# kieranrcampbell/clonealign

Measured on AMD Instinct MI355X. Metric: ELBO iterations/sec, higher is better.
Workload: dtype f32 variables (contraction: float64 series over gene bins; count-matrix products: int8 MFMA, exact); 1 GPU; synthetic 100000 cells x 5000 genes x 8 clones, K=1, S=1, cell-sharded over 1 GPU(s) (BASELINE.json configs[2]); cells=100000, genes=5000, clones=8, K=1, mc_samples=1, y_storage=u8, y_bytes_per_elem=1, fused_sweep=True, fwd_mfma=True, series_form=True, y_mfma=True, parallelism=single, collective=none, allreduce_doubles_per_train_pass=20764, build_id=88308988739b5500

## Files before the change

clonealign_amd/csrc/ca_eng_loop.inc:

```
int wait_y(ca_engine* h, bool all) {
  if (all) {
    if (h->y_pending) HIPCK(h, hipStreamWaitEvent(h->stream, h->ev_ydone, 0));
    h->y_pending = false; h->yw_pending = false;
  } else if (h->yw_pending) {
    HIPCK(h, hipStreamWaitEvent(h->stream, h->ev_ywdone, 0));
    h->yw_pending = false;
  }
  return CA_OK;
}

int make_etamax(ca_engine* h) {
  if (h->D > 0) {
    LAUNCH(h, CA_KERNEL_OTHER, hipLaunchKernelGGL(k_vmm_final, dim3(1), dim3(64), 0, h->stream, h->vmm_part, h->vmm, h->ngblk, h->D));
    LAUNCH(h, CA_KERNEL_OTHER, hipLaunchKernelGGL(k_etamax, dim3(cdiv(h->N, CA_TB)), dim3(CA_TB), 0, h->stream, h->F, h->vmm, h->etamax2, h->N, h->D));
  }
  h->em_stale = false;
  return CA_OK;
}
int ensure_etamax(ca_engine* h) {
  if (!h->em_stale) return CA_OK;
  return make_etamax(h);
}

int refresh_derived(ca_engine* h) {
// ... 69 lines not shown
                                                  h->V, h->D, (int64_t)h->G, h->F, h->D, h->N, 1, h->ys_amax));
  }
  LAUNCH(h, CA_KERNEL_OTHER, hipLaunchKernelGGL(k_ys_quant, dim3(a.nblk), dim3(CA_YM_TB), 0, h->stream, a));
  return CA_OK;
}
ca_ys_io ys_io(ca_engine* h) {
  ca_ys_io io;
  io.Wr = h->Wr; io.Pr = h->Pr; io.Wsum = h->Wsum; io.Psum = h->Psum; io.exps = h->ys_exps + 2 * h->ys_slot;
  io.YWpart = h->YWpart; io.YTpart = h->YTpart;
  io.esc_off = h->ys4 ? h->esc_off : nullptr; io.esc = h->ys4 ? h->esc : nullptr;
  io.perm = nullptr;
  return io;
}
ca_ovf_args ys_ovf(ca_engine* h) { return ovf_args(h, h->YWpart + (int64_t)h->ys_nseg * h->N); }
int yfin_flush(ca_engine* h) {
  if (!h->yfin_pending) return CA_OK;
  h->yfin_pending = false;
  return launch_yfinish(h, h->ys_nrg, h->ys_nseg);
}
int ys_finish(ca_engine* h, bool defer = false) {
  h->yfin_pending = true;
  if (!defer) CACK(yfin_flush(h));
  h->ys_slot = (h->ys_slot + 1) % 3;
  h->ys_steps = 0;
  h->ys_quant_ready = false;
  h->ycache_valid = true;
  return CA_OK;
}
template <bool Y4, int N2 = 0>
void launch_ys(ca_engine* h) {
  constexpr int lds = Y4 ? CA_YS4_LDS_BYTES : CA_YS_LDS_BYTES;
  ca_ys_io yio = ys_io(h);
  const uint8_t* Yimg = h->Ys;
  if (N2 > 0) { Yimg = h->Ys2; yio.esc_off = h->esc2_off; yio.esc = h->esc2; yio.perm = h->y2_perm; }
  const int nb_main = h->ys_nrg * h->ys_nseg;
  const ca_pm_args* pm = h->mom_args;
  h->mom_args = nullptr;
  const int nmom = pm ? pm->nmb + pm->nred : 0;
  if (h->n_ovf > 0) {
    const ca_ovf_args ovf = ys_ovf(h);
    const dim3 grid(nmom + nb_main + ovf.nb_rows + ovf.nb_chunks);
    if (pm) {
      ca_pm_args pmo = *pm;
      if (h->mom_last && h->mom_ovf_first) pmo.blk0 += ovf.nb_rows + ovf.nb_chunks;
      hipLaunchKernelGGL((k_ys_mfma_ovf_mom<Y4, N2>), grid, dim3(CA_YM_TB), lds, h->stream, Yimg, yio, h->N, h->Gp, h->ys_RS, nb_main, ovf, h->F, h->V, h->D, pmo);
    }
// ... 847 lines not shown
```

clonealign_amd/csrc/ca_eng_state.inc:

```
namespace {

thread_local std::string g_last_error;

typedef struct { char internal[128]; } ca_nccl_uid;
typedef void* ca_nccl_comm;
struct RcclApi {
  void* lib = nullptr;
  int (*GetUniqueId)(ca_nccl_uid*) = nullptr;
  int (*CommInitRank)(ca_nccl_comm*, int, ca_nccl_uid, int) = nullptr;
  int (*CommDestroy)(ca_nccl_comm) = nullptr;
  int (*AllReduce)(const void*, void*, size_t, int, int, ca_nccl_comm, hipStream_t) = nullptr;
  const char* (*GetErrorString)(int) = nullptr;
  std::string err;
  bool load() {
    if (lib) return true;
    const char* cands[] = {getenv("CLONEALIGN_RCCL_LIB"), "librccl.so.1", "librccl.so", "/opt/rocm/lib/librccl.so.1",
                           "/opt/rocm/lib/librccl.so"};
    for (const char* c : cands) {
      if (!c || !*c) continue;
      lib = dlopen(c, RTLD_NOW | RTLD_LOCAL);
      if (lib) break;
    }
    if (!lib) { err = std::string("cannot dlopen librccl: ") + dlerror(); return false; }
    GetUniqueId = (decltype(GetUniqueId))dlsym(lib, "ncclGetUniqueId");
// ... 130 lines not shown
  bool tail_fuse = true;
  double* host_dev = nullptr;
  unsigned long long host_seq = 0, host_seq_next = 0;
  float* eps_stage = nullptr; size_t eps_stage_bytes = 0;
  hipEvent_t ev_stage = nullptr;
  bool fwd_cell = false; int ncblk_f = 0, fc_tl = 4;
  int fc_nbig = 0;
  bool fwd_mfma = false; int fsplit = 1, fkchunk = 1, nk32 = 1; unsigned short* Mq = nullptr;
  bool fwd_bal = false; int bal_q = 0, bal_r = 0, bal_nchunk = 0; unsigned long long* bal_xw = nullptr; unsigned bal_tag = 0;
  bool pfwd = false; int pf_npair = 0, pf_fsplit = 1, pf_kchunk = 1; unsigned short* pf_Mq = nullptr; float* pf_Z = nullptr;
  int bwd_pairs = 0;
  bool bwd_mfma = false, bwd_frac = false, c16 = false, s2 = false, s2f = false;
  unsigned short* coefq = nullptr; int64_t N16 = 0, cchunk_m = 0; int csplit_m = 1, nwt = 0;
  int bwd_tl = CA_BWD_TL;
  uint64_t draw = 0;
  hipEvent_t ev_ywdone = nullptr; bool yw_pending = false, on_side = false;
  bool y_ys = false, ys4 = false; int* esc_off = nullptr; unsigned* esc = nullptr; int64_t n_esc = 0;
  int ys_n2 = 0; uint8_t* Ys2 = nullptr; unsigned short *y2_perm = nullptr, *y2_pos = nullptr; int* esc2_off = nullptr; unsigned* esc2 = nullptr; int64_t n_esc2 = 0;
  uint8_t* Ys = nullptr; uint4 *Wr = nullptr, *Pr = nullptr; int *Wsum = nullptr, *Psum = nullptr;
  int* ys_exps = nullptr;
  unsigned* ys_amax = nullptr;
  float* ys_amaxp = nullptr; int ys_nq = 0;
  int ys_ncap = 0, ys_namax[3] = {0, 0, 0};
  bool ys_quant_ready = false;
  int ys_slot = 0, ys_steps = -1, ys_RS = 256, ys_nrg = 0, ys_nseg = 0; int64_t ys_N64 = 0; float ys_step_bound = -1.f;
  double adam_bound = -1.0;
  ca_p2p* p2p = nullptr;
  ca_nccl_comm comm = nullptr;
  ca_host_allreduce_fn host_ar = nullptr; void* host_ar_user = nullptr; double* host_ar_buf = nullptr; int64_t host_ar_cap = 0;
  std::vector<EvPair> ev_pool; size_t ev_used = 0; bool prof_open = false;
  unsigned prof_seen[CA_KERNEL_COUNT] = {0, 0, 0, 0, 0};
  double k_ms[CA_KERNEL_COUNT] = {0}; int64_t k_n[CA_KERNEL_COUNT] = {0};
  int n_cu = 256;
};

namespace {

#define HIPCK(h, call)                                                                       \
  do {                                                                                       \
    hipError_t e_ = (call);                                                                  \
    if (e_ != hipSuccess) {                                                                  \
      (h)->err = std::string(#call) + ": " + hipGetErrorString(e_);                          \
      return CA_ERR_HIP;                                                                     \
    }                                                                                        \
  } while (0)

// ... 321 lines not shown
```

clonealign_amd/csrc/ca_ymfma.hip.h:

```cpp
#pragma once
#include <hip/hip_runtime.h>
#include <stdint.h>

typedef int ca_i32x4 __attribute__((ext_vector_type(4)));

#define CA_YM_TB 256

__device__ __forceinline__ int ca_fix_exp(float amax) { return amax > 0.f ? 29 - ilogbf(amax) : 0; }

__global__ void __launch_bounds__(CA_YM_TB) k_ym_absmax(const float* __restrict__ V, int Dv, int64_t G, const float* __restrict__ F, int Df,
                                                        int64_t N, int K, unsigned* __restrict__ amax) {
  const int64_t i = (int64_t)blockIdx.x * CA_YM_TB + threadIdx.x;
  float mw = 0.f, mp = 0.f;
  if (i < G) for (int k = 0; k < K; ++k) mw = fmaxf(mw, fabsf(V[i * Dv + k]));
  if (i < N) for (int k = 0; k < K; ++k) mp = fmaxf(mp, fabsf(F[i * Df + k]));
#pragma unroll
  for (int o = 32; o > 0; o >>= 1) { mw = fmaxf(mw, __shfl_xor(mw, o, 64)); mp = fmaxf(mp, __shfl_xor(mp, o, 64)); }
  if ((threadIdx.x & 63) == 0) {
    if (i < G + 64) atomicMax(amax, __float_as_uint(mw));
    if (i < N + 64) atomicMax(amax + 1, __float_as_uint(mp));
  }
}
__device__ __forceinline__ int ca_digit(int x, int p) {
  int d = 0;
// ... 162 lines not shown
        const unsigned y = n < N ? col[n * (int64_t)Gp] : 0u;
        x |= (y < 3u ? y : 3u) << (2 * t);
      }
    } else {
#pragma unroll
      for (int t = 0; t < 2; ++t) {
        const int64_t n = cs * 64 + 32 * ld + 16 * t + j;
        const unsigned y = n < N ? col[n * (int64_t)Gp] : 0u;
        x |= (y < 15u ? y : 15u) << (4 * t);
      }
    }
    w[gb >> 2] |= x << (8 * (gb & 3));
  }
  Y2[i] = (uint4){w[0], w[1], w[2], w[3]};
}

__device__ __forceinline__ ca_i32x4 ca_mfma_i8(uint4 a, uint4 b, ca_i32x4 c) {
  return __builtin_amdgcn_mfma_i32_16x16x64_i8(__builtin_bit_cast(ca_i32x4, a), __builtin_bit_cast(ca_i32x4, b), c, 0, 0, 0);
}

constexpr int CA_YS_GW = 512;
static_assert(CA_YS_GW == 512, "k_ys_mfma's accumulator switch has eight cases");
constexpr int CA_YS_PITCH = 80;

__device__ __forceinline__ void ca_ds_read_tr_b8_x8(unsigned addr, uint2 (&lo)[4], uint2 (&hi)[4]) {
  asm volatile(
      "ds_read_b64_tr_b8 %0, %8\n\tds_read_b64_tr_b8 %4, %8 offset:640\n\t"
      "ds_read_b64_tr_b8 %1, %8 offset:16\n\tds_read_b64_tr_b8 %5, %8 offset:656\n\t"
      "ds_read_b64_tr_b8 %2, %8 offset:32\n\tds_read_b64_tr_b8 %6, %8 offset:672\n\t"
      "ds_read_b64_tr_b8 %3, %8 offset:48\n\tds_read_b64_tr_b8 %7, %8 offset:688\n\t"
      "s_waitcnt lgkmcnt(0)"
      : "=&v"(lo[0]), "=&v"(lo[1]), "=&v"(lo[2]), "=&v"(lo[3]), "=&v"(hi[0]), "=&v"(hi[1]), "=&v"(hi[2]), "=&v"(hi[3])
      : "v"(addr)
      : "memory");
}
__device__ __forceinline__ void ca_ds_read_tr_b8_x4(unsigned addr, uint2 (&lo)[2], uint2 (&hi)[2]) {
  asm volatile(
      "ds_read_b64_tr_b8 %0, %4\n\tds_read_b64_tr_b8 %2, %4 offset:640\n\t"
      "ds_read_b64_tr_b8 %1, %4 offset:16\n\tds_read_b64_tr_b8 %3, %4 offset:656\n\t"
      "s_waitcnt lgkmcnt(0)"
      : "=&v"(lo[0]), "=&v"(lo[1]), "=&v"(hi[0]), "=&v"(hi[1])
      : "v"(addr)
      : "memory");
}
static_assert(8 * CA_YS_PITCH == 640, "offsets in ca_ds_read_tr_b8_x8 / _x4 assume the 80-byte pitch");
__device__ __forceinline__ uint4 ca_and4(uint4 a, unsigned m) { return (uint4){a.x & m, a.y & m, a.z & m, a.w & m}; }

#ifndef CA_YS_DEPTH
#define CA_YS_DEPTH 2
#endif
#ifndef CA_YS_WAVES
#define CA_YS_WAVES 3
#endif
struct ca_ys_io {
  const uint4* Wr; const uint4* Pr; const int* Wsum; const int* Psum; const int* exps;
  float* YWpart; float* YTpart;
  const int* esc_off; const unsigned* esc;
  const unsigned short* perm;
};
#ifndef CA_YS4_DEPTH
#define CA_YS4_DEPTH 4
#endif
#ifndef CA_YS4_WAVES
#define CA_YS4_WAVES 4
#endif
constexpr int CA_YS4_OFF_W = 4 * 64 * CA_YS_PITCH;
constexpr int CA_YS4_OFF_ROW = CA_YS4_OFF_W + (CA_YS_GW / 64) * 1024;
constexpr int CA_YS4_OFF_PSI = CA_YS4_OFF_ROW + 4 * 64 * 8;
constexpr int CA_YS4_OFF_COL = 4 * (CA_YS_GW / 64) * 64 * 4 * 4;
constexpr int CA_YS4_LDS_BYTES = CA_YS4_OFF_COL + CA_YS_GW * 8;
static_assert(CA_YS4_OFF_PSI + 4 * 256 <= CA_YS4_OFF_COL, "the 4-bit launch's tables fit below its column-escape sums");
static_assert(4 * CA_YS4_LDS_BYTES <= 160 * 1024, "four blocks of the 4-bit launch per CU");
template <int DEPTH = CA_YS_DEPTH, bool Y4 = false, bool OWN = false, int N2 = 0>
__device__ __forceinline__ void ca_ys_mfma_body(int blk, const uint8_t* __restrict__ Ys, const ca_ys_io& io, int64_t N, int Gp,
                                                int RS ,
                                                unsigned char* ca_ys_lds ) {
  const uint4* __restrict__ Wr = io.Wr;
  const uint4* __restrict__ Pr = io.Pr;
  constexpr bool Y4L = Y4 && OWN;
  constexpr int NP = CA_YS_GW / 64;
  static_assert(NP % DEPTH == 0, "pieces per cell step must be a multiple of the pipeline depth");
  static_assert(N2 == 0 || (Y4 && OWN && N2 < NP), "the 2-bit blocks belong to the 4-bit image's own launch");
  constexpr int SB2 = N2 * 1024 + (NP - N2) * 2048;
  const int lane = threadIdx.x & 63, j = lane & 15, q = lane >> 4;
  const int wv = __builtin_amdgcn_readfirstlane((int)(threadIdx.x >> 6) & 3);
  const int nseg = Gp / CA_YS_GW;
  const int rg = blk / nseg, seg = blk - rg * nseg;
  unsigned char* my = ca_ys_lds + (size_t)wv * 64 * CA_YS_PITCH;
  const int64_t c0 = ((int64_t)rg * 4 + wv) * RS;
  const int64_t c1 = (c0 + RS < N) ? c0 + RS : N;
  const int g0 = seg * CA_YS_GW;
  const unsigned grp = (unsigned)(j >> 2);
  unsigned msk[4];
#pragma unroll
  for (int t = 0; t < 4; ++t) msk[t] = grp == (unsigned)t ? 0xFFFFFFFFu : 0u;
  ca_i32x4 acc_yt[NP];
#pragma unroll
  for (int a = 0; a < NP; ++a) acc_yt[a] = (ca_i32x4){0, 0, 0, 0};
  const int lrow = lane >> 2, lch = lane & 3;
  unsigned char* wr_dst = my + lrow * CA_YS_PITCH + 16 * lch;
  const unsigned char* rd_row = my + j * CA_YS_PITCH + 16 * q;
  const unsigned rd_tr = (unsigned)(size_t)my + (unsigned)((16 * q + (j >> 1)) * CA_YS_PITCH + 8 * (j & 1));
  constexpr int PB = Y4 ? 2048 : 4096, NL = PB / 1024;
  const uint8_t* src = N2 > 0 ? Ys + ((c0 >> 6) * (int64_t)nseg + seg) * SB2
                              : Ys + ((c0 >> 6) * (int64_t)(Gp / 64) + (g0 >> 6)) * PB;
  const uint4* wsrc = Wr + (int64_t)(g0 >> 6) * 64;
  const unsigned voff = 16u * (unsigned)lane;
  uint4 R[DEPTH][NL], W[DEPTH];
  const int nsteps = c0 < c1 ? (int)((c1 - c0 + 63) / 64) : 0;
  typedef unsigned ca_v4u __attribute__((ext_vector_type(4)));
  const __amdgpu_buffer_rsrc_t ry = __builtin_amdgcn_make_buffer_rsrc(const_cast<uint8_t*>(src), 0, 0x7FFFFFFF, 0x00020000);
  const __amdgpu_buffer_rsrc_t rw = __builtin_amdgcn_make_buffer_rsrc(const_cast<uint4*>(wsrc), 0, NP * 1024, 0x00020000);
  const __amdgpu_buffer_rsrc_t rp = __builtin_amdgcn_make_buffer_rsrc(const_cast<uint4*>(Pr + (c0 >> 6) * 64), 0, 0x7FFFFFFF, 0x00020000);
  auto issue = [&](int slot, int st, int a, unsigned vo) {
    const int so = N2 > 0 ? st * nseg * SB2 + (a < N2 ? a * 1024 : N2 * 1024 + (a - N2) * 2048) : (st * (Gp / 64) + a) * PB;
#pragma unroll
    for (int i = 0; i < NL; ++i) {
      if (N2 > 0 && i > 0 && a < N2) continue;
      const ca_v4u v = __builtin_amdgcn_raw_buffer_load_b128(ry, (int)(vo + 1024u * (unsigned)i), so, 2 );
      R[slot][i] = (uint4){v.x, v.y, v.z, v.w};
    }
    if (!Y4L) {
      const ca_v4u w = __builtin_amdgcn_raw_buffer_load_b128(rw, (int)voff, a * 1024, 0);
      W[slot] = (uint4){w.x, w.y, w.z, w.w};
    }
  };
  uint4* wl = reinterpret_cast<uint4*>(ca_ys_lds + CA_YS4_OFF_W);
  unsigned long long* colesc = reinterpret_cast<unsigned long long*>(ca_ys_lds + CA_YS4_OFF_COL);
  uint4 wimg[2], pidx[2][2];
  int eoff = 0;
  if (Y4L) {
    wimg[0] = wsrc[threadIdx.x];
    wimg[1] = wsrc[threadIdx.x + CA_YM_TB];
    if (N2 > 0) {
#pragma unroll
      for (int h2 = 0; h2 < 2; ++h2) {
        const uint4* pq = reinterpret_cast<const uint4*>(io.perm + g0 + 16 * (((int)threadIdx.x + h2 * CA_YM_TB) >> 4));
        pidx[h2][0] = pq[0]; pidx[h2][1] = pq[1];
      }
    }
    if (lane <= nsteps) eoff = io.esc_off[((int64_t)blk * 4 + wv) * RS + (64 * lane < RS ? 64 * lane : RS)];
  }
// ... 25 lines not shown
          w4[b >> 2] |= (unsigned)tb[((gi >> 6) * 64 + 16 * ((gi >> 4) & 3)) * 16 + (gi & 15)] << (8 * (b & 3));
        }
        wimg[h2] = (uint4){w4[0], w4[1], w4[2], w4[3]};
      }
    }
    wl[threadIdx.x] = wimg[0];
    wl[threadIdx.x + CA_YM_TB] = wimg[1];
    colesc[threadIdx.x] = 0ull;
    colesc[threadIdx.x + CA_YM_TB] = 0ull;
    __syncthreads();
  }
  ca_i32x4 acc_yw[4];
  uint4 prm[4];
  int wtot[4] = {0, 0, 0, 0};
  if (!Y4) {
    const int* ws = io.Wsum + (g0 >> 6) * 4;
#pragma unroll
    for (int a = 0; a < NP; ++a)
#pragma unroll
      for (int p_ = 0; p_ < 4; ++p_) wtot[p_] += ws[a * 4 + p_];
  }
  const int e_w = io.exps[0];
  const int64_t kb = ((int64_t)blk * 4 + wv) * RS;
  unsigned long long* rowesc = reinterpret_cast<unsigned long long*>(ca_ys_lds + (Y4L ? CA_YS4_OFF_ROW : 4 * 64 * CA_YS_PITCH)) + wv * 64;
  unsigned char* psl = ca_ys_lds + CA_YS4_OFF_PSI + wv * 256;
  if (Y4) rowesc[lane] = 0ull;
  for (int st = 0; st < nsteps; ++st) {
    const int64_t cs = c0 + (int64_t)st * 64;
    const bool more = st + 1 < nsteps;
    uint4 pr;
    if (Y4L) {
      pr = pr_nx;
#pragma unroll
      for (int t = 0; t < 4; ++t) acc_yw[t] = (ca_i32x4){0, 0, 0, 0};
    } else {
      const ca_v4u pv = __builtin_amdgcn_raw_buffer_load_b128(rp, (int)voff, st * 1024, 0);
      pr = (uint4){pv.x, pv.y, pv.z, pv.w};
#pragma unroll
      for (int t = 0; t < 4; ++t) { acc_yw[t] = (ca_i32x4){0, 0, 0, 0}; if (!Y4L) prm[t] = ca_and4(pr, msk[t]); }
    }
    int e_lo = 0, e_hi = 0;
    unsigned en0 = 0u, en1 = 0u;
    if (Y4L) {
      e_lo = __builtin_amdgcn_readlane(eoff, st);
      e_hi = __builtin_amdgcn_readlane(eoff, st + 1);
      if (e_hi > e_lo) {
        en0 = io.esc[e_lo + lane < e_hi ? e_lo + lane : e_hi - 1];
        en1 = io.esc[e_lo + 64 + lane < e_hi ? e_lo + 64 + lane : e_hi - 1];
      }
    }
#pragma unroll
    for (int a = 0; a < NP; ++a) {
      const int slot = a % DEPTH;
      __builtin_amdgcn_sched_barrier(0);
      const uint4 wr = Y4L ? wl[a * 64 + lane] : W[slot];
      if (Y4) {
#pragma unroll
        for (int t = 0; t < 4; ++t) {
          const bool nar = N2 > 0 && a < N2;
          const uint4 v = R[slot][nar ? 0 : t >> 1];
          const int sh = nar ? 2 * t : 4 * (t & 1);
          const uint4 av = ca_and4((uint4){v.x >> sh, v.y >> sh, v.z >> sh, v.w >> sh}, nar ? 0x03030303u : 0x0F0F0F0Fu);
          *reinterpret_cast<uint4*>(const_cast<unsigned char*>(rd_row) + 16 * t * CA_YS_PITCH) = av;
          acc_yw[t] = ca_mfma_i8(av, wr, acc_yw[t]);
        }
        if (a + DEPTH < NP) issue(slot, st, a + DEPTH, voff);
        else if (Y4L) {
          const unsigned vo = more ? voff : 0x80000000u + voff;
          if (a + DEPTH == NP) {
            const ca_v4u pv = __builtin_amdgcn_raw_buffer_load_b128(rp, (int)vo, (st + 1) * 1024, 0);
            pr_nx = (uint4){pv.x, pv.y, pv.z, pv.w};
          }
          issue(slot, st + 1, a + DEPTH - NP, vo);
        } else if (more) issue(slot, st + 1, a + DEPTH - NP, voff);
      } else {
#pragma unroll
        for (int i = 0; i < 4; ++i) *reinterpret_cast<uint4*>(wr_dst + 16 * i * CA_YS_PITCH) = R[slot][i];
        if (a + DEPTH < NP) issue(slot, st, a + DEPTH, voff);
        else if (more) issue(slot, st + 1, a + DEPTH - NP, voff);
#pragma unroll
        for (int t = 0; t < 4; ++t) {
          const uint4 av = *reinterpret_cast<const uint4*>(rd_row + 16 * t * CA_YS_PITCH);
          acc_yw[t] = ca_mfma_i8(av, wr, acc_yw[t]);
        }
      }
#pragma unroll
      for (int h2 = 0; h2 < 2; ++h2) {
        uint2 lo[2], hi[2];
        ca_ds_read_tr_b8_x4(rd_tr + 32u * (unsigned)h2, lo, hi);
#pragma unroll
        for (int t = 0; t < 2; ++t) {
          uint4 pa;
          if (Y4L) {
            unsigned g_ = grp;
            asm volatile("" : "+v"(g_));
            pa = ca_and4(pr, g_ == (unsigned)(2 * h2 + t) ? 0xFFFFFFFFu : 0u);
          } else {
            pa = prm[2 * h2 + t];
          }
          acc_yt[a] = ca_mfma_i8(pa, (uint4){lo[t].x, lo[t].y, hi[t].x, hi[t].y}, acc_yt[a]);
        }
      }
    }
    if (Y4L) {
      if (j < 4) *reinterpret_cast<uint4*>(psl + (4 * q + j) * 16) = pr;
      const unsigned char* wlb = reinterpret_cast<const unsigned char*>(wl);
      auto esc1 = [&](unsigned en) {
        const int c = (int)(en & 63u), gi = (int)((en >> 9) & 511u);
        const unsigned char* dw = wlb + ((gi >> 6) * 64 + 16 * ((gi >> 4) & 3)) * 16 + (gi & 15);
        const unsigned char* dp = psl + 64 * (c >> 4) + (c & 15);
        unsigned fw = 0u, fp = 0u;
#pragma unroll
        for (int p_ = 0; p_ < 4; ++p_) {
          fw += (unsigned)(int)(signed char)dw[16 * p_] << (8 * p_);
          fp += (unsigned)(int)(signed char)dp[16 * p_] << (8 * p_);
        }
        const long long x = (long long)(en >> 18);
        atomicAdd(rowesc + c, (unsigned long long)(x * (long long)(int)fw));
        atomicAdd(colesc + gi, (unsigned long long)(x * (long long)(int)fp));
// ... 60 lines not shown
    }
  }
  const double inv_p = ldexp(1.0, -io.exps[1]);
  for (int i = (int)threadIdx.x & (CA_YM_TB - 1); i < NP * 64; i += CA_YM_TB) {
    const int l = i & 63, a = i >> 6;
    double v = 0.0;
#pragma unroll
    for (int r = 3; r >= 0; --r) {
      const int o = i * 4 + r;
      const int sr = (comb[o] + comb[o + NP * 256]) + (comb[o + 2 * NP * 256] + comb[o + 3 * NP * 256]);
      v = v * 256.0 + (double)((long long)sr + 128 * pb[r]);
    }
    const int gl = 16 * (4 * a + (l >> 4)) + (l & 15), gene = g0 + (N2 > 0 ? (int)io.perm[g0 + gl] : gl);
    if (Y4L) v += (double)(long long)colesc[gl];
    io.YTpart[(int64_t)rg * Gp + gene] = (float)(v * inv_p);
  }
}
template <bool Y4, int N2 = 0>
__global__ void __launch_bounds__(CA_YM_TB, Y4 ? CA_YS4_WAVES : CA_YS_WAVES) k_ys_mfma(const uint8_t* __restrict__ Ys, ca_ys_io io, int64_t N, int Gp, int RS) {
  extern __shared__ __attribute__((aligned(16))) unsigned char ca_ys_dyn[];
  ca_ys_mfma_body<Y4 ? CA_YS4_DEPTH : CA_YS_DEPTH, Y4, true, N2>((int)blockIdx.x, Ys, io, N, Gp, RS, ca_ys_dyn);
}
constexpr int CA_YS_LDS_BYTES = 4 * (CA_YS_GW / 64) * 64 * 4 * 4;
static_assert(4 * 64 * CA_YS_PITCH + 4 * 64 * 8 <= CA_YS_LDS_BYTES, "staging + row escapes fit the combine buffer");

struct ca_ysq_args {
  int nblk;
  const float* V; int Dv; int64_t G; int GS; const float* F; int Df; int64_t N; int64_t NS;
  const float* amax_in; int n_in; float slack_w, slack_p;
  float* amax_out;
  int* exps; uint4* Wr; uint4* Pr; int* Wsum; int* Psum;
};
__device__ __forceinline__ void ca_ys_quant_core(const ca_ysq_args& a, bool live, bool isw, int64_t step, const float (&vals)[16], float own,
                                                 int out, bool write_exps, float* sm ) {
  const int tid = threadIdx.x, l = tid & 63, wv = tid >> 6;
  float mw = 0.f, mp = 0.f;
  for (int i = tid; i < a.n_in; i += CA_YM_TB) { mw = fmaxf(mw, a.amax_in[2 * i]); mp = fmaxf(mp, a.amax_in[2 * i + 1]); }
#pragma unroll
  for (int o = 32; o > 0; o >>= 1) { mw = fmaxf(mw, __shfl_xor(mw, o, 64)); mp = fmaxf(mp, __shfl_xor(mp, o, 64)); }
  if (l == 0) { sm[2 * wv] = mw; sm[2 * wv + 1] = mp; }
  __syncthreads();
  mw = fmaxf(fmaxf(sm[0], sm[2]), fmaxf(sm[4], sm[6]));
  mp = fmaxf(fmaxf(sm[1], sm[3]), fmaxf(sm[5], sm[7]));
  __syncthreads();
  const int ew = ca_fix_exp(mw + a.slack_w), ep = ca_fix_exp(mp + a.slack_p);
  if (write_exps && tid == 0) { a.exps[0] = ew; a.exps[1] = ep; }
  float m = 0.f;
// ... 102 lines not shown
```

clonealign_amd/csrc/clonealign_hip.hip:

```cpp
#include "clonealign_hip.h"

#include <dlfcn.h>
#include <unistd.h>
#include <hip/hip_runtime.h>

#include <algorithm>
#include <cmath>
#include <cstdio>
#include <cstring>
#include <string>
#include <atomic>
#include <chrono>
#include <thread>
#include <vector>

#include "ca_kernels.hip.h"
#include "ca_poly.h"
#include "philox_host.h"

#include "ca_eng_state.inc"
#include "ca_eng_launch.inc"
#include "ca_eng_reduce.inc"
#include "ca_eng_loop.inc"
#include "ca_eng_ingest.inc"
// ... 596 lines not shown
    for (int64_t i = 0; i < r.rows; ++i) se += std::exp((double)buf[i] - mx);
    for (int64_t i = 0; i < r.rows; ++i) out[i] = std::exp((double)buf[i] - mx - std::log(se));
    return CA_OK;
  }
  for (int64_t i = 0; i < r.rows; ++i) {
    for (int64_t c = 0; c < r.cols; ++c) row[c] = (double)buf[i * r.stride + r.off + c];
    if (r.xform == 1) for (auto& x : row) x = x > 0 ? x + std::log1p(std::exp(-x)) : std::log1p(std::exp(x));
    if (r.xform == 3) for (auto& x : row) x = std::exp(x);
    if (r.xform == 2) {
      double mx = -INFINITY, se = 0.0;
      for (int64_t c = 0; c < r.cols; ++c) mx = std::max(mx, row[c]);
      for (int64_t c = 0; c < r.cols; ++c) se += std::exp(row[c] - mx);
      const double lse = mx + std::log(se);
      for (int64_t c = 0; c < r.cols; ++c) row[c] = std::exp(row[c] - lse);
    }
    for (int64_t c = 0; c < r.cols; ++c) out[r.matrix ? hidx(h->layout, i, c, r.rows, r.cols) : i] = row[c];
  }
  return CA_OK;
}

int ca_get_param(ca_handle h, const char* name, double* out) { return get_generic(h, name, out, false); }
int ca_get_gradient(ca_handle h, const char* name, double* out) { return get_generic(h, name, out, true); }

int ca_set_param(ca_handle h, const char* name, const double* in) {
  if (!h || !name || !in) return CA_ERR_INVALID;
  CA_NOT_IN_RUN(h);
  HIPCK(h, hipSetDevice(h->device));
  ParamRef r;
  if (!find_param(h, name, false, r) || r.xform != 0 || r.d) { h->err = std::string("cannot set parameter: ") + name; return CA_ERR_INVALID; }
  if (r.rows * r.cols == 0) return CA_OK;
  std::vector<float> buf;
  CACK(download_f(h, buf, r.f, r.rows * std::max<int64_t>(r.stride, 1)));
  for (int64_t i = 0; i < r.rows; ++i)
    for (int64_t c = 0; c < r.cols; ++c)
      buf[i * r.stride + r.off + c] = (float)in[r.matrix ? hidx(h->layout, i, c, r.rows, r.cols) : i];
  CACK(upload_f(h, r.f, buf));
  CACK(refresh_derived(h));
  SYNC(h);
  return CA_OK;
}

int ca_reinit(ca_handle h, const double* psi0, const double* loc0) {
  if (!h) return CA_ERR_INVALID;
  CA_NOT_IN_RUN(h);
  if (h->K > 0 && !psi0) { h->err = "psi0 is required when K > 0"; return CA_ERR_INVALID; }
  HIPCK(h, hipSetDevice(h->device));
// ... 145 lines not shown
```

clonealign_amd/engine.py:

```python
import ctypes as C
import os

import numpy as np

from . import hostprep

_HERE = os.path.dirname(os.path.abspath(__file__))
LIB_PATH = os.path.join(_HERE, "libclonealign_hip.so")

CA_OK = 0
CA_ERR_NAN = 4
CA_INTERRUPTED = 7
CA_ABI_VERSION = 6
P2P_HANDLE_BYTES = 128
CA_F64, CA_F32, CA_I32, CA_U16, CA_U8 = 0, 1, 2, 3, 4
CA_ROW_MAJOR, CA_COL_MAJOR = 0, 1
YSTORE = {"auto": 0, "f32": 1, "u16": 2, "u8": 3}
YSTORE_NAME = {v: k for k, v in YSTORE.items()}
KERNEL_NAMES = ("fwd", "bwd", "ypass", "cell", "other")
VARIANTS = {"fused": 1 << 0, "fwd_mfma": 1 << 1, "fwd_cell": 1 << 2, "bwd_mfma": 1 << 3, "tail_fuse": 1 << 4, "async_y": 1 << 5,
            "pre": 1 << 6, "pair_elbo": 1 << 7, "prep_fast": 1 << 8, "update_merge": 1 << 9, "p2p": 1 << 10, "fold_gsum": 1 << 11, "y_ride": 1 << 12, "ride_seq": 1 << 13, "y_mfma1": 1 << 14, "yfin_ride": 1 << 15, "p2p_ride": 1 << 16, "run_gate": 1 << 17, "s2_fuse": 1 << 18, "fwd_bal": 1 << 19, "bwd_tl3": 1 << 20, "series": 1 << 21, "y4": 1 << 22, "mom_ride": 1 << 23, "cell_lean": 1 << 24, "mom_last": 1 << 25, "cell_mfma": 1 << 26, "y2": 1 << 27}
VARIANTS_ON = {"y_mfma2": 1 << 0, "async_small": 1 << 1, "y_mfma1": 1 << 2, "fold_always": 1 << 3, "ride_seq": 1 << 4, "p2p_same_device": 1 << 5, "run_fwd": 1 << 6, "bal_tiles": 1 << 7, "series": 1 << 8, "y4": 1 << 9, "mom_last": 1 << 10, "y2": 1 << 11}
OPT_VERBOSE = 0x80000000
TUNE = {"gsplit": 0, "fsplit": 1, "fc_tl": 2, "fc_nbig": 3, "csplit": 4, "csplit_m": 5, "tr": 6, "rg": 7}
TRANSPORT_NAME = {0: "none", 1: "rccl", 2: "host", 3: "p2p"}

EXPORTS = (
    "ca_abi_version", "ca_build_id", "ca_device_count", "ca_default_options", "ca_create", "ca_destroy", "ca_last_error", "ca_get_info",
    "ca_synchronize", "ca_stream_busy", "ca_comm_unique_id", "ca_comm_init", "ca_p2p_export", "ca_p2p_connect", "ca_p2p_commit", "ca_comm_benchmark", "ca_comm_selftest", "ca_set_host_allreduce", "ca_gamma_init", "ca_elbo", "ca_elbo_terms",
    "ca_step", "ca_gradients", "ca_run", "ca_run_ex", "ca_iterate", "ca_final_elbo", "ca_init_psi_pca", "ca_clone_gene_sums", "ca_get_param", "ca_set_param",
    "ca_get_gradient", "ca_reinit", "ca_get_kernel_times", "ca_reset_kernel_times", "ca_set_profile", "ca_eps_draw", "ca_allele_loglik", "ca_preprocess",
    "ca_group_create", "ca_group_destroy", "ca_group_last_error", "ca_group_get_info", "ca_group_rank_handle", "ca_group_init_psi_pca", "ca_group_gamma_init",
    "ca_group_elbo", "ca_group_step", "ca_group_run_ex", "ca_group_iterate", "ca_group_final_elbo", "ca_group_get_param", "ca_group_reinit",
    "ca_group_clone_gene_sums",
    "ca_create_sparse", "ca_group_create_sparse",
    "ca_fit_mse", "ca_group_fit_mse",
    "ca_logexpr_sums", "ca_group_logexpr_sums",
    "ca_clone_loglik", "ca_group_clone_loglik",
    "ca_project_cells", "ca_group_project_cells",
    "ca_clone_pair_loglik", "ca_group_clone_pair_loglik",
    "ca_clone_loglik_dm", "ca_group_clone_loglik_dm",
    "ca_clone_loglik_by_block", "ca_group_clone_loglik_by_block",
    "ca_simulate_counts", "ca_simulate_kernel_ms",
    "ca_predictive_stats", "ca_predictive_kernel_ms",
    "ca_predictive_moments", "ca_predictive_moments_kernel_ms",
    "ca_clone_evidence", "ca_group_clone_evidence",
    "ca_clone_loglik_reweighted", "ca_group_clone_loglik_reweighted", "ca_reweighted_kernel_ms",
)
CA_BOOT_RCHUNK = 32


def reweighted_cells_per_batch(n, G, C, D, R):
    rc = min(int(R), CA_BOOT_RCHUNK)
    nzc, nw = -(-int(G) // 512), -(-int(C) // 32)
    nc1, nc2 = -(-rc * (C + 1) // 16) * 16, -(-rc * C // 16) * 16
    per_cell = (nzc * (nc1 + (nc2 + 1 if D > 0 else 0)) + rc * (C + 1) + 2 * C) * 8 + (rc * nw + C) * 4
    return min(int(n), max(256, ((1 << 28) // per_cell) // 256 * 256))
CA_SPARSE_CSR, CA_SPARSE_CSC = 0, 1


class CaProblem(C.Structure):
    _fields_ = [("N", C.c_int64), ("G", C.c_int32), ("C", C.c_int32), ("K", C.c_int32), ("P", C.c_int32),
                ("S", C.c_int32), ("layout", C.c_int32), ("y_dtype", C.c_int32), ("y_on_device", C.c_int32),
                ("Y", C.c_void_p), ("L", C.c_void_p), ("psi0", C.c_void_p), ("loc0", C.c_void_p),
                ("X", C.c_void_p), ("extra_loglik", C.c_void_p),
                ("N_src", C.c_int64), ("G_src", C.c_int32), ("cell_index", C.c_void_p), ("gene_index", C.c_void_p),
                ("y_ld", C.c_int64)]


class CaSparse(C.Structure):
# ... 50 lines not shown
        return _lib
    p = path or os.environ.get("CLONEALIGN_HIP_LIB") or LIB_PATH
    if not os.path.exists(p):
        raise RuntimeError(
            f"{p} not found: build the HIP engine first (python -c 'import __graft_entry__ as g; g.build()' "
            "or make -C clonealign_amd/csrc). clonealign_amd has no CPU fallback.")
    lib = C.CDLL(p)
    lib.ca_last_error.restype = C.c_char_p
    lib.ca_last_error.argtypes = [C.c_void_p]
    lib.ca_build_id.restype = C.c_char_p
    lib.ca_build_id.argtypes = []
    lib.ca_group_last_error.restype = C.c_char_p
    lib.ca_group_last_error.argtypes = [C.c_void_p]
    for name in EXPORTS:
        if name not in ("ca_last_error", "ca_build_id", "ca_group_last_error"):
            getattr(lib, name).restype = C.c_int
    lib.ca_device_count.argtypes = [C.POINTER(C.c_int32)]
    lib.ca_create.argtypes = [C.POINTER(CaProblem), C.POINTER(CaOptions), C.POINTER(C.c_void_p)]
    lib.ca_create_sparse.argtypes = [C.POINTER(CaProblem), C.POINTER(CaSparse), C.POINTER(CaOptions), C.POINTER(C.c_void_p)]
    lib.ca_destroy.argtypes = [C.c_void_p]
    lib.ca_get_info.argtypes = [C.c_void_p, C.POINTER(CaInfo)]
    lib.ca_synchronize.argtypes = [C.c_void_p]
    lib.ca_stream_busy.argtypes = [C.c_void_p, C.POINTER(C.c_int32)]
    lib.ca_comm_unique_id.argtypes = [C.c_char_p]
    lib.ca_comm_init.argtypes = [C.c_void_p, C.c_char_p]
    lib.ca_p2p_export.argtypes = [C.c_void_p, C.c_char_p]
    lib.ca_p2p_connect.argtypes = [C.c_void_p, C.c_char_p]
    lib.ca_p2p_commit.argtypes = [C.c_void_p, C.c_int32]
    lib.ca_comm_benchmark.argtypes = [C.c_void_p, C.c_int32, C.c_int32, C.c_int64, C.POINTER(C.c_double)]
    lib.ca_comm_selftest.argtypes = [C.c_void_p, C.c_int32, C.c_int64, C.POINTER(C.c_int64)]
    lib.ca_set_host_allreduce.argtypes = [C.c_void_p, HOST_ALLREDUCE_FN, C.c_void_p]
    lib.ca_gamma_init.argtypes = [C.c_void_p, C.c_void_p]
    lib.ca_elbo.argtypes = [C.c_void_p, C.c_void_p, C.POINTER(C.c_double)]
    lib.ca_elbo_terms.argtypes = [C.c_void_p, C.c_void_p, C.POINTER(C.c_double)]
    lib.ca_step.argtypes = [C.c_void_p, C.c_void_p]
    lib.ca_gradients.argtypes = [C.c_void_p, C.c_void_p, C.POINTER(C.c_double)]
    lib.ca_run.argtypes = [C.c_void_p, C.c_int32, C.c_double, C.c_void_p, C.c_int64, C.c_void_p,
                           C.POINTER(C.c_int32)]
    lib.ca_run_ex.argtypes = [C.c_void_p, C.c_int32, C.c_double, C.c_void_p, C.c_int64, C.c_void_p,
                              C.POINTER(C.c_int32), POLL_FN, C.c_void_p]
    lib.ca_iterate.argtypes = [C.c_void_p, C.c_int32, C.c_void_p, C.c_int64, C.POINTER(C.c_double)]
    lib.ca_final_elbo.argtypes = [C.c_void_p, C.c_int32, C.c_void_p, C.c_int64, C.c_void_p,
                                  C.POINTER(C.c_double), C.POINTER(C.c_double)]
    lib.ca_init_psi_pca.argtypes = [C.c_void_p, C.c_void_p, C.c_int32, C.c_uint64, C.c_void_p]
    lib.ca_clone_gene_sums.argtypes = [C.c_void_p, C.c_void_p, C.c_void_p, C.c_void_p]
    lib.ca_fit_mse.argtypes = [C.c_void_p, C.c_void_p, C.c_void_p, C.POINTER(C.c_double), C.POINTER(C.c_int64), C.c_void_p, C.c_void_p]
# ... 609 lines not shown
        nd = np.ascontiguousarray(nodes, dtype=np.float64)
        Q = int(wts.shape[0])
        if nd.size != Q * max(K, 0):
            raise ValueError(f"clone_evidence: nodes is {nd.shape}; {Q} weights and K = {K} need ({Q}, {K})")
        Kp = max(K, 0)
        NH = Kp * (Kp + 1) // 2
        ev, lap, mode, prec = self._zeros(self.N, self.C), self._zeros(self.N, self.C), self._zeros(self.N, self.C * Kp), self._zeros(self.N, self.C * NH)
        rounds = np.zeros((self.N, self.C), dtype=np.int32, order=self._order)
        conv = np.zeros((self.N, self.C), dtype=np.uint8, order=self._order)
        Em, Vm, Xm, psm, nd_p, wts_p, *outs = (_ptr(a, empty_null=True) for a in (Em, Vm, Xm, psm, nd, wts, ev, lap, mode, prec, rounds, conv))
        self._ck(self._fn("clone_evidence")(self.h, Em, Vm, K, P, Xm, psm, flags, Q, nd_p, wts_p, int(max_iter), float(tol), float(max_step), *outs))
        return {"evidence": np.ascontiguousarray(ev), "laplace": np.ascontiguousarray(lap), "psi_mode": np.ascontiguousarray(mode).reshape(self.N, self.C, Kp),
                "psi_prec": np.ascontiguousarray(prec).reshape(self.N, self.C, NH), "rounds": np.ascontiguousarray(rounds),
                "converged": np.ascontiguousarray(conv).astype(bool)}

    def synchronize(self):
        self._ck(self.lib.ca_synchronize(self.h))

    def stream_busy(self):
        b = C.c_int32()
        self._ck(self.lib.ca_stream_busy(self.h, C.byref(b)))
        return bool(b.value)

    def _shape(self, name):
        N, G, Cn, K, P = self.N, self.G, self.C, self.K, self.P
        return {"mu": (G,), "loc": (G,), "ls": (G,), "clone_probs": (N, Cn), "gamma_logits": (N, Cn), "s": (N,),
                "alpha": (Cn,), "alpha_unconstr": (Cn,), "beta": (G, P), "psi": (N, K), "W": (G, K),
                "chi": (K,), "v": (K,)}[name]

    def _get(self, fn, name):
        out = np.zeros(self._shape(name), dtype=np.float64, order=self._order)
        if out.size:
            self._ck(fn(self.h, name.encode(), out.ctypes.data_as(C.c_void_p)))
        return out

    def get(self, name):
        return self._get(self._fn("get_param"), name)

    def set(self, name, value):
        v = np.require(np.asarray(value, dtype=np.float64).reshape(self._shape(name)), requirements=[self._order, "A"])
        if v.size:
            self._ck(self.lib.ca_set_param(self.h, name.encode(), v.ctypes.data_as(C.c_void_p)))

    def reinit(self, psi0, loc0=None):
        p0 = None
        if self.K > 0:
# ... 265 lines not shown
```

include/clonealign_hip.h:

```cpp
#ifndef CLONEALIGN_HIP_H
#define CLONEALIGN_HIP_H

#include <stdint.h>

#ifdef __cplusplus
extern "C" {
#endif

#define CA_ABI_VERSION 6

typedef struct ca_engine* ca_handle;

enum ca_status {
  CA_OK = 0,
  CA_ERR_INVALID = 1,
  CA_ERR_HIP = 2,
  CA_ERR_NOMEM = 3,
  CA_ERR_NAN = 4,
  CA_ERR_COMM = 5,
  CA_ERR_STATE = 6,
  CA_INTERRUPTED = 7
};

enum ca_dtype { CA_F64 = 0, CA_F32 = 1, CA_I32 = 2, CA_U16 = 3, CA_U8 = 4 };
// ... 140 lines not shown
int ca_device_count(int32_t* n);
int ca_default_options(ca_options* opts);

int ca_create(const ca_problem* problem, const ca_options* opts, ca_handle* out);

enum ca_sparse_kind { CA_SPARSE_CSR = 0,
                      CA_SPARSE_CSC = 1 };
typedef struct ca_sparse {
  int32_t kind;
  int32_t val_dtype;
  int32_t index_bytes;
  int32_t on_device;
  int64_t nnz;
  const void* ptr;
  const void* idx;
  const void* val;
} ca_sparse;
int ca_create_sparse(const ca_problem* problem, const ca_sparse* y, const ca_options* opts, ca_handle* out);
int ca_destroy(ca_handle h);
const char* ca_last_error(ca_handle h);
int ca_get_info(ca_handle h, ca_info* info);
int ca_synchronize(ca_handle h);
int ca_stream_busy(ca_handle h, int32_t* busy);

int ca_comm_unique_id(char id[128]);
int ca_comm_init(ca_handle h, const char id[128]);
#define CA_P2P_HANDLE_BYTES 128
int ca_p2p_export(ca_handle h, char handle[CA_P2P_HANDLE_BYTES]);
int ca_p2p_connect(ca_handle h, const char* handles );
int ca_p2p_commit(ca_handle h, int32_t all_ranks_ok);
int ca_comm_benchmark(ca_handle h, int32_t transport, int32_t n_calls, int64_t n_doubles, double* us_per_call);
int ca_comm_selftest(ca_handle h, int32_t n_rounds, int64_t n_doubles, int64_t* n_bad);
typedef int (*ca_host_allreduce_fn)(void* user, double* buf, int64_t n);
int ca_set_host_allreduce(ca_handle h, ca_host_allreduce_fn fn, void* user);

int ca_gamma_init(ca_handle h, const float* eps);
int ca_elbo(ca_handle h, const float* eps, double* elbo);
int ca_elbo_terms(ca_handle h, const float* eps, double terms[3]);
int ca_step(ca_handle h, const float* eps);
int ca_gradients(ca_handle h, const float* eps, double* elbo);

int ca_run(ca_handle h, int32_t max_iter, double rel_tol, const float* eps_stream, int64_t n_draws,
           double* elbo_trace, int32_t* n_elbo);
typedef int (*ca_poll_fn)(void* user, int32_t iter, double elbo);
int ca_run_ex(ca_handle h, int32_t max_iter, double rel_tol, const float* eps_stream, int64_t n_draws,
              double* elbo_trace, int32_t* n_elbo, ca_poll_fn poll, void* user);
// ... 157 lines not shown
```

Before: 10050 iterations/s.

## Pad LDS cell tiles to avoid bank conflicts in count-matrix MFMA stream

Restructures the per-wave LDS staging in the u8 count-matrix MFMA kernel so each 16-row cell tile gets an extra 128-byte pad, putting odd tiles 32 banks away from even ones. The goal is to reduce bank conflicts on the transposed ds_read and on the staging writes. It also changes the buffer-load cache policy for the 4-bit path and replaces the opaque group-mask compare with a v_bfe_i32 extract. A debugging API, ca_ystream_parts, is added to read back partial sums and fixed-point images. The larger staging footprint shifts LDS offsets, which could affect occupancy.

```diff
diff --git a/clonealign_amd/csrc/ca_eng_loop.inc b/clonealign_amd/csrc/ca_eng_loop.inc
--- a/clonealign_amd/csrc/ca_eng_loop.inc
+++ b/clonealign_amd/csrc/ca_eng_loop.inc
@@ -115,6 +115,7 @@
   h->yfin_pending = true;
   if (!defer) CACK(yfin_flush(h));
   h->ys_slot = (h->ys_slot + 1) % 3;
+  h->ys_launched = true;
   h->ys_steps = 0;
   h->ys_quant_ready = false;
   h->ycache_valid = true;
diff --git a/clonealign_amd/csrc/ca_eng_state.inc b/clonealign_amd/csrc/ca_eng_state.inc
--- a/clonealign_amd/csrc/ca_eng_state.inc
+++ b/clonealign_amd/csrc/ca_eng_state.inc
@@ -176,6 +176,7 @@
   unsigned* ys_amax = nullptr;
   float* ys_amaxp = nullptr; int ys_nq = 0;
   int ys_ncap = 0, ys_namax[3] = {0, 0, 0};
+  bool ys_launched = false;
   bool ys_quant_ready = false;
   int ys_slot = 0, ys_steps = -1, ys_RS = 256, ys_nrg = 0, ys_nseg = 0; int64_t ys_N64 = 0; float ys_step_bound = -1.f;
   double adam_bound = -1.0;
diff --git a/clonealign_amd/csrc/ca_ymfma.hip.h b/clonealign_amd/csrc/ca_ymfma.hip.h
--- a/clonealign_amd/csrc/ca_ymfma.hip.h
+++ b/clonealign_amd/csrc/ca_ymfma.hip.h
@@ -208,6 +208,9 @@
 constexpr int CA_YS_GW = 512;
 static_assert(CA_YS_GW == 512, "k_ys_mfma's accumulator switch has eight cases");
 constexpr int CA_YS_PITCH = 80;
+constexpr int CA_YS_TILE = 16 * CA_YS_PITCH + 128;
+constexpr int CA_YS_STAGE = 4 * CA_YS_TILE;
+static_assert((CA_YS_TILE / 4) % 64 == 32 && CA_YS_TILE % 16 == 0, "odd cell tiles sit 32 banks off the even ones, 16-byte aligned");
 
 __device__ __forceinline__ void ca_ds_read_tr_b8_x8(unsigned addr, uint2 (&lo)[4], uint2 (&hi)[4]) {
   asm volatile(
@@ -229,7 +232,7 @@
       : "v"(addr)
       : "memory");
 }
-static_assert(8 * CA_YS_PITCH == 640, "offsets in ca_ds_read_tr_b8_x8 / _x4 assume the 80-byte pitch");
+static_assert(8 * CA_YS_PITCH == 640, "offsets in ca_ds_read_tr_b8_x8 / _x4 assume the 80-byte pitch inside a cell tile (rows 8 .. 15 of the tile the lane's address names)");
 __device__ __forceinline__ uint4 ca_and4(uint4 a, unsigned m) { return (uint4){a.x & m, a.y & m, a.z & m, a.w & m}; }
 
 #ifndef CA_YS_DEPTH
@@ -250,12 +253,13 @@
 #ifndef CA_YS4_WAVES
 #define CA_YS4_WAVES 4
 #endif
-constexpr int CA_YS4_OFF_W = 4 * 64 * CA_YS_PITCH;
+constexpr int CA_YS4_OFF_W = 4 * CA_YS_STAGE;
 constexpr int CA_YS4_OFF_ROW = CA_YS4_OFF_W + (CA_YS_GW / 64) * 1024;
 constexpr int CA_YS4_OFF_PSI = CA_YS4_OFF_ROW + 4 * 64 * 8;
-constexpr int CA_YS4_OFF_COL = 4 * (CA_YS_GW / 64) * 64 * 4 * 4;
+constexpr int CA_YS4_COMB = 4 * (CA_YS_GW / 64) * 64 * 4 * 4;
+constexpr int CA_YS4_OFF_COL = CA_YS4_OFF_PSI + 4 * 256 > CA_YS4_COMB ? CA_YS4_OFF_PSI + 4 * 256 : CA_YS4_COMB;
 constexpr int CA_YS4_LDS_BYTES = CA_YS4_OFF_COL + CA_YS_GW * 8;
-static_assert(CA_YS4_OFF_PSI + 4 * 256 <= CA_YS4_OFF_COL, "the 4-bit launch's tables fit below its column-escape sums");
+static_assert(CA_YS4_OFF_PSI + 4 * 256 <= CA_YS4_OFF_COL && CA_YS4_COMB <= CA_YS4_OFF_COL, "the 4-bit launch's tables and the combine buffer lie below its column-escape sums");
 static_assert(4 * CA_YS4_LDS_BYTES <= 160 * 1024, "four blocks of the 4-bit launch per CU");
 template <int DEPTH = CA_YS_DEPTH, bool Y4 = false, bool OWN = false, int N2 = 0>
 __device__ __forceinline__ void ca_ys_mfma_body(int blk, const uint8_t* __restrict__ Ys, const ca_ys_io& io, int64_t N, int Gp,
@@ -272,7 +276,7 @@
   const int wv = __builtin_amdgcn_readfirstlane((int)(threadIdx.x >> 6) & 3);
   const int nseg = Gp / CA_YS_GW;
   const int rg = blk / nseg, seg = blk - rg * nseg;
-  unsigned char* my = ca_ys_lds + (size_t)wv * 64 * CA_YS_PITCH;
+  unsigned char* my = ca_ys_lds + (size_t)wv * CA_YS_STAGE;
   const int64_t c0 = ((int64_t)rg * 4 + wv) * RS;
   const int64_t c1 = (c0 + RS < N) ? c0 + RS : N;
   const int g0 = seg * CA_YS_GW;
@@ -280,13 +284,14 @@
   unsigned msk[4];
 #pragma unroll
   for (int t = 0; t < 4; ++t) msk[t] = grp == (unsigned)t ? 0xFFFFFFFFu : 0u;
+  const unsigned gsel = 0xFFu << (8u * grp);
   ca_i32x4 acc_yt[NP];
 #pragma unroll
   for (int a = 0; a < NP; ++a) acc_yt[a] = (ca_i32x4){0, 0, 0, 0};
   const int lrow = lane >> 2, lch = lane & 3;
   unsigned char* wr_dst = my + lrow * CA_YS_PITCH + 16 * lch;
   const unsigned char* rd_row = my + j * CA_YS_PITCH + 16 * q;
-  const unsigned rd_tr = (unsigned)(size_t)my + (unsigned)((16 * q + (j >> 1)) * CA_YS_PITCH + 8 * (j & 1));
+  const unsigned rd_tr = (unsigned)(size_t)my + (unsigned)(q * CA_YS_TILE + (j >> 1) * CA_YS_PITCH + 8 * (j & 1));
   constexpr int PB = Y4 ? 2048 : 4096, NL = PB / 1024;
   const uint8_t* src = N2 > 0 ? Ys + ((c0 >> 6) * (int64_t)nseg + seg) * SB2
                               : Ys + ((c0 >> 6) * (int64_t)(Gp / 64) + (g0 >> 6)) * PB;
@@ -303,7 +308,7 @@
 #pragma unroll
     for (int i = 0; i < NL; ++i) {
       if (N2 > 0 && i > 0 && a < N2) continue;
-      const ca_v4u v = __builtin_amdgcn_raw_buffer_load_b128(ry, (int)(vo + 1024u * (unsigned)i), so, 2 );
+      const ca_v4u v = __builtin_amdgcn_raw_buffer_load_b128(ry, (int)(vo + 1024u * (unsigned)i), so, Y4L ? 0 : 2 );
       R[slot][i] = (uint4){v.x, v.y, v.z, v.w};
     }
     if (!Y4L) {
@@ -375,7 +380,7 @@
   }
   const int e_w = io.exps[0];
   const int64_t kb = ((int64_t)blk * 4 + wv) * RS;
-  unsigned long long* rowesc = reinterpret_cast<unsigned long long*>(ca_ys_lds + (Y4L ? CA_YS4_OFF_ROW : 4 * 64 * CA_YS_PITCH)) + wv * 64;
+  unsigned long long* rowesc = reinterpret_cast<unsigned long long*>(ca_ys_lds + (Y4L ? CA_YS4_OFF_ROW : 4 * CA_YS_STAGE)) + wv * 64;
   unsigned char* psl = ca_ys_lds + CA_YS4_OFF_PSI + wv * 256;
   if (Y4) rowesc[lane] = 0ull;
   for (int st = 0; st < nsteps; ++st) {
@@ -414,7 +419,7 @@
           const uint4 v = R[slot][nar ? 0 : t >> 1];
           const int sh = nar ? 2 * t : 4 * (t & 1);
           const uint4 av = ca_and4((uint4){v.x >> sh, v.y >> sh, v.z >> sh, v.w >> sh}, nar ? 0x03030303u : 0x0F0F0F0Fu);
-          *reinterpret_cast<uint4*>(const_cast<unsigned char*>(rd_row) + 16 * t * CA_YS_PITCH) = av;
+          *reinterpret_cast<uint4*>(const_cast<unsigned char*>(rd_row) + t * CA_YS_TILE) = av;
           acc_yw[t] = ca_mfma_i8(av, wr, acc_yw[t]);
         }
         if (a + DEPTH < NP) issue(slot, st, a + DEPTH, voff);
@@ -428,12 +433,12 @@
         } else if (more) issue(slot, st + 1, a + DEPTH - NP, voff);
       } else {
 #pragma unroll
-        for (int i = 0; i < 4; ++i) *reinterpret_cast<uint4*>(wr_dst + 16 * i * CA_YS_PITCH) = R[slot][i];
+        for (int i = 0; i < 4; ++i) *reinterpret_cast<uint4*>(wr_dst + i * CA_YS_TILE) = R[slot][i];
         if (a + DEPTH < NP) issue(slot, st, a + DEPTH, voff);
         else if (more) issue(slot, st + 1, a + DEPTH - NP, voff);
 #pragma unroll
         for (int t = 0; t < 4; ++t) {
-          const uint4 av = *reinterpret_cast<const uint4*>(rd_row + 16 * t * CA_YS_PITCH);
+          const uint4 av = *reinterpret_cast<const uint4*>(rd_row + t * CA_YS_TILE);
           acc_yw[t] = ca_mfma_i8(av, wr, acc_yw[t]);
         }
       }
@@ -445,9 +450,9 @@
         for (int t = 0; t < 2; ++t) {
           uint4 pa;
           if (Y4L) {
-            unsigned g_ = grp;
-            asm volatile("" : "+v"(g_));
-            pa = ca_and4(pr, g_ == (unsigned)(2 * h2 + t) ? 0xFFFFFFFFu : 0u);
+            unsigned m_;
+            asm volatile("v_bfe_i32 %0, %1, %2, 8" : "=v"(m_) : "v"(gsel), "n"(8 * (2 * h2 + t)));
+            pa = ca_and4(pr, m_);
           } else {
             pa = prm[2 * h2 + t];
           }
@@ -554,7 +559,7 @@
   ca_ys_mfma_body<Y4 ? CA_YS4_DEPTH : CA_YS_DEPTH, Y4, true, N2>((int)blockIdx.x, Ys, io, N, Gp, RS, ca_ys_dyn);
 }
 constexpr int CA_YS_LDS_BYTES = 4 * (CA_YS_GW / 64) * 64 * 4 * 4;
-static_assert(4 * 64 * CA_YS_PITCH + 4 * 64 * 8 <= CA_YS_LDS_BYTES, "staging + row escapes fit the combine buffer");
+static_assert(4 * CA_YS_STAGE + 4 * 64 * 8 <= CA_YS_LDS_BYTES, "staging + row escapes fit the combine buffer");
 
 struct ca_ysq_args {
   int nblk;
diff --git a/clonealign_amd/csrc/clonealign_hip.hip b/clonealign_amd/csrc/clonealign_hip.hip
--- a/clonealign_amd/csrc/clonealign_hip.hip
+++ b/clonealign_amd/csrc/clonealign_hip.hip
@@ -642,6 +642,34 @@
 int ca_get_param(ca_handle h, const char* name, double* out) { return get_generic(h, name, out, false); }
 int ca_get_gradient(ca_handle h, const char* name, double* out) { return get_generic(h, name, out, true); }
 
+int ca_ystream_parts(ca_handle h, int64_t dims[6], float* yw_part, float* yt_part, int32_t exps[2], int32_t* w_fix, int32_t* p_fix) {
+  if (!h || !dims) return CA_ERR_INVALID;
+  if (!h->y_ys || h->K != 1) { h->err = "ca_ystream_parts: this engine does not run the one-copy count-matrix stream"; return CA_ERR_INVALID; }
+  if (!h->ys_launched) { h->err = "ca_ystream_parts: no launch of the count-matrix stream yet (ca_elbo / ca_gradients / a loop call makes one)"; return CA_ERR_STATE; }
+  HIPCK(h, hipSetDevice(h->device));
+  CACK(gate_close(h));
+  CACK(wait_y(h, true));
+  const int64_t N = h->N, Gp = h->Gp, N64 = h->ys_N64;
+  dims[0] = h->ys_nseg; dims[1] = N; dims[2] = h->ys_nrg; dims[3] = Gp; dims[4] = h->ys_RS;
+  dims[5] = (h->ycache_valid && !h->ys_quant_ready) ? 1 : 0;
+  if (yw_part) HIPCK(h, hipMemcpyAsync(yw_part, h->YWpart, (size_t)(h->ys_nseg * N) * sizeof(float), hipMemcpyDeviceToHost, h->stream));
+  if (yt_part) HIPCK(h, hipMemcpyAsync(yt_part, h->YTpart, (size_t)(h->ys_nrg * Gp) * sizeof(float), hipMemcpyDeviceToHost, h->stream));
+  if (exps) HIPCK(h, hipMemcpyAsync(exps, h->ys_exps + 2 * ((h->ys_slot + 2) % 3), 2 * sizeof(int32_t), hipMemcpyDeviceToHost, h->stream));
+  std::vector<signed char> wi(w_fix ? (size_t)Gp * 16 : 0), pi(p_fix ? (size_t)N64 * 16 : 0);
+  if (w_fix) HIPCK(h, hipMemcpyAsync(wi.data(), h->Wr, wi.size(), hipMemcpyDeviceToHost, h->stream));
+  if (p_fix) HIPCK(h, hipMemcpyAsync(pi.data(), h->Pr, pi.size(), hipMemcpyDeviceToHost, h->stream));
+  SYNC(h);
+  auto fix = [](const std::vector<signed char>& img, int64_t n, int32_t* out) {
+    for (int64_t i = 0; i < n; ++i) {
+      const signed char* d = img.data() + ((i >> 6) * 64 + 16 * ((i >> 4) & 3)) * 16 + (i & 15);
+      out[i] = (int32_t)((int64_t)d[0] + (int64_t)d[16] * 256 + (int64_t)d[32] * 65536 + (int64_t)d[48] * 16777216);
+    }
+  };
+  if (w_fix) fix(wi, Gp, w_fix);
+  if (p_fix) fix(pi, N64, p_fix);
+  return CA_OK;
+}
+
 int ca_set_param(ca_handle h, const char* name, const double* in) {
   if (!h || !name || !in) return CA_ERR_INVALID;
   CA_NOT_IN_RUN(h);
diff --git a/clonealign_amd/engine.py b/clonealign_amd/engine.py
--- a/clonealign_amd/engine.py
+++ b/clonealign_amd/engine.py
@@ -46,6 +46,7 @@
     "ca_predictive_moments", "ca_predictive_moments_kernel_ms",
     "ca_clone_evidence", "ca_group_clone_evidence",
     "ca_clone_loglik_reweighted", "ca_group_clone_loglik_reweighted", "ca_reweighted_kernel_ms",
+    "ca_ystream_parts",
 )
 CA_BOOT_RCHUNK = 32
 
@@ -142,6 +143,7 @@
     lib.ca_get_info.argtypes = [C.c_void_p, C.POINTER(CaInfo)]
     lib.ca_synchronize.argtypes = [C.c_void_p]
     lib.ca_stream_busy.argtypes = [C.c_void_p, C.POINTER(C.c_int32)]
+    lib.ca_ystream_parts.argtypes = [C.c_void_p, C.POINTER(C.c_int64), C.c_void_p, C.c_void_p, C.c_void_p, C.c_void_p, C.c_void_p]
     lib.ca_comm_unique_id.argtypes = [C.c_char_p]
     lib.ca_comm_init.argtypes = [C.c_void_p, C.c_char_p]
     lib.ca_p2p_export.argtypes = [C.c_void_p, C.c_char_p]
@@ -797,6 +799,16 @@
         self._ck(self.lib.ca_stream_busy(self.h, C.byref(b)))
         return bool(b.value)
 
+    def ystream_parts(self):
+        dims = (C.c_int64 * 6)()
+        self._ck(self.lib.ca_ystream_parts(self.h, dims, None, None, None, None, None))
+        nseg, N, nrg, Gp, RS, _cur = (int(d) for d in dims)
+        N64 = -(-N // 64) * 64
+        yw, yt = np.empty((nseg, N), np.float32), np.empty((nrg, Gp), np.float32)
+        exps, wf, pf = np.empty(2, np.int32), np.empty(Gp, np.int32), np.empty(N64, np.int32)
+        self._ck(self.lib.ca_ystream_parts(self.h, dims, *(a.ctypes.data_as(C.c_void_p) for a in (yw, yt, exps, wf, pf))))
+        return {"yw_part": yw, "yt_part": yt, "exps": exps, "w_fix": wf, "p_fix": pf, "strip_cells": RS, "images_current": bool(dims[5])}
+
     def _shape(self, name):
         N, G, Cn, K, P = self.N, self.G, self.C, self.K, self.P
         return {"mu": (G,), "loc": (G,), "ls": (G,), "clone_probs": (N, Cn), "gamma_logits": (N, Cn), "s": (N,),
diff --git a/include/clonealign_hip.h b/include/clonealign_hip.h
--- a/include/clonealign_hip.h
+++ b/include/clonealign_hip.h
@@ -186,6 +186,7 @@
 int ca_get_info(ca_handle h, ca_info* info);
 int ca_synchronize(ca_handle h);
 int ca_stream_busy(ca_handle h, int32_t* busy);
+int ca_ystream_parts(ca_handle h, int64_t dims[6], float* yw_part, float* yt_part, int32_t exps[2], int32_t* w_fix, int32_t* p_fix);
 
 int ca_comm_unique_id(char id[128]);
 int ca_comm_init(ca_handle h, const char id[128]);
```

New measurement: 10300 iterations/s (median of 6 runs). 2.5% higher.
